# hkbharath/MARL-MASS

Hardware: AMD Instinct MI355X
Metric: agent-steps/sec (whole node), MASS CBF shield on, 65536 envs x 8 CAVs (higher is better)
Workload: dtype f64

## Files before the change

### include/mm_qp.h

```cpp
#ifndef MM_QP_H
#define MM_QP_H

#ifndef MMM_FN
#define MMM_FN static inline
#endif

#define MM_QP_MAXITERS 100
#define MM_QP_ABSTOL 1e-7
#define MM_QP_RELTOL 1e-6
#define MM_QP_FEASTOL 1e-7
#define MM_QP_STEP 0.99
#define MM_QP_FEASTOL_SQ 0x1.6849b86a12b9bp-47

#ifndef MM_QP_RCP
#define MM_QP_RCP(b) (b)
#define MM_QP_DIVR(a, b, R) ((a) / (b))
#endif
#ifndef MM_QP_DIV
#define MM_QP_DIV(a, b) ((a) / (b))
#endif
#ifndef MM_QP_SQRT
#define MM_QP_SQRT(x) sqrt(x)
#endif

typedef struct MMQpKkt {
  double g0, g3;
  double l00, l20, l22;
  double r00, r22;
  double di0, di1, di2, di3;
} MMQpKkt;

typedef struct MMQpState {
  double a, h0, h1, h2, h3, resz0;
  double x0, x2, gap;
  double s0, s1, s2, s3, z0, z1, z2, z3;
  double d0, d1, d2, d3, di0, di1, di2, di3;
  double l0, l1, l2, l3;
  double ax0, ax2;
  int m4, iters;
} MMQpState;
typedef struct MMQpRes { double rx0, rx2, rz0, rz1, rz2, rz3; } MMQpRes;

MMM_FN int mm_qp_factor(MMQpKkt *f, double a, int m4, double di0, double di1, double di2, double di3) {
  f->di0 = di0; f->di1 = di1; f->di2 = di2; f->di3 = 0.0;
  f->g0 = di0 * a;
  f->g3 = 0.0;
  double s00 = f->g0 * f->g0 + di1 * di1 + di2 * di2;
  double s20 = 0.0 + (-di0) * f->g0;
  double s22 = di0 * di0;
  if (m4) {
    f->di3 = di3;
    f->g3 = di3 * a;
    s00 = s00 + f->g3 * f->g3;
    s20 = s20 + (-di3) * f->g3;
    s22 = s22 + di3 * di3;
  }
  s00 = s00 + 1.0;
  s22 = s22 + 1e18;
  if (!(s00 > 0.0)) return 0;
  f->l00 = MM_QP_SQRT(s00);
  f->r00 = MM_QP_RCP(f->l00);
  f->l20 = MM_QP_DIVR(s20, f->l00, f->r00);
  const double t = s22 - f->l20 * f->l20;
  if (!(t > 0.0)) return 0;
  f->l22 = MM_QP_SQRT(t);
  f->r22 = MM_QP_RCP(f->l22);
  return 1;
}
MMM_FN void mm_qp_solve(const MMQpKkt *f, int m4, double *x0, double *x2, double *z0, double *z1, double *z2, double *z3) {
  double w0 = *z0 * f->di0, w1 = *z1 * f->di1, w2 = *z2 * f->di2, w3 = 0.0;
  double t = 0.0 + f->g0 * w0;
  t = t + f->di1 * w1;
  t = t + (-f->di2) * w2;
  double u = 0.0 + (-f->di0) * w0;
  if (m4) {
    w3 = *z3 * f->di3;
    t = t + f->g3 * w3;
    u = u + (-f->di3) * w3;
  }
  double a0 = *x0 + t;
  double a2 = *x2 + u;
  a0 = MM_QP_DIVR(a0, f->l00, f->r00);
  a2 = a2 - a0 * f->l20;
  a2 = MM_QP_DIVR(a2, f->l22, f->r22);
  a2 = MM_QP_DIVR(a2, f->l22, f->r22);
  t = a0 - f->l20 * a2;
  a0 = MM_QP_DIVR(t, f->l00, f->r00);
  t = -w0; t = t + a0 * f->g0; t = t + a2 * (-f->di0); *z0 = t;
  t = -w1; t = t + a0 * f->di1; *z1 = t;
  t = -w2; t = t + a0 * (-f->di2); *z2 = t;
  if (m4) { t = -w3; t = t + a0 * f->g3; t = t + a2 * (-f->di3); *z3 = t; }
  *x0 = a0; *x2 = a2;
}
MMM_FN double mm_qp_dot(double p0, double q0, double p1, double q1, double p2, double q2, double p3, double q3, int m4) {
  double t = 0.0 + p0 * q0;
  t = t + p1 * q1;
  t = t + p2 * q2;
  if (m4) t = t + p3 * q3;
  return t;
}
MMM_FN double mm_qp_maxneg(double p0, double p1, double p2, double p3, int m4) {
  double t = -p0;
  if (-p1 > t) t = -p1;
  if (-p2 > t) t = -p2;
  if (m4 && -p3 > t) t = -p3;
  return t;
}

MMM_FN int mm_qp_start(MMQpState *q, double a, double h0, double h1, double h2, double h3, int rows) {
  const int m4 = rows == 4;
  q->a = a; q->m4 = m4; q->iters = 0;
  q->ax0 = q->ax2 = INFINITY;
  q->h0 = h0; q->h1 = h1; q->h2 = h2; q->h3 = m4 ? h3 : 0.0;
  q->resz0 = fmax(1.0, sqrt(mm_qp_dot(q->h0, q->h0, q->h1, q->h1, q->h2, q->h2, q->h3, q->h3, m4)));
  q->d0 = q->d1 = q->d2 = q->d3 = 1.0; q->di0 = q->di1 = q->di2 = q->di3 = 1.0; q->l0 = q->l1 = q->l2 = q->l3 = 1.0;
  MMQpKkt kkt;
  if (!mm_qp_factor(&kkt, a, m4, 1.0, 1.0, 1.0, 1.0)) {
    q->x0 = a - a + (h0 - h0); q->x2 = q->x0; q->gap = q->x0;
    q->s0 = q->s1 = q->s2 = q->s3 = q->z0 = q->z1 = q->z2 = q->z3 = q->x0;
    return 0;
  }
  double x0 = -0.0, x2 = -0.0;
  double z0 = q->h0, z1 = q->h1, z2 = q->h2, z3 = q->h3;
  mm_qp_solve(&kkt, m4, &x0, &x2, &z0, &z1, &z2, &z3);
  double s0 = -z0, s1 = -z1, s2 = -z2, s3 = -z3;
  const double ts = mm_qp_maxneg(s0, s1, s2, s3, m4);
  int shift = ts >= 0.0;
  if (!shift) shift = ts >= -1e-8 * fmax(sqrt(mm_qp_dot(s0, s0, s1, s1, s2, s2, s3, s3, m4)), 1.0);
  if (shift) { const double sh = 1.0 + ts; s0 = s0 + sh; s1 = s1 + sh; s2 = s2 + sh; s3 = s3 + sh; }
  const double tz = mm_qp_maxneg(z0, z1, z2, z3, m4);
  shift = tz >= 0.0;
  if (!shift) shift = tz >= -1e-8 * fmax(sqrt(mm_qp_dot(z0, z0, z1, z1, z2, z2, z3, z3, m4)), 1.0);
  if (shift) { const double sh = 1.0 + tz; z0 = z0 + sh; z1 = z1 + sh; z2 = z2 + sh; z3 = z3 + sh; }
  q->x0 = x0; q->x2 = x2;
  q->s0 = s0; q->s1 = s1; q->s2 = s2; q->s3 = s3; q->z0 = z0; q->z1 = z1; q->z2 = z2; q->z3 = z3;
  q->gap = mm_qp_dot(s0, z0, s1, z1, s2, z2, s3, z3, m4);
  return 1;
}

#ifndef MM_QP_ILOGB
#define MM_QP_ILOGB(x) ilogb(x)
#define MM_QP_LDEXP(x, e) ldexp(x, e)
#define MM_QP_RINT(x) rint(x)
#endif
MMM_FN int mm_qp_row_state(double s, double z, double rz, double hmag) {
  if (rz == 0.0 && s <= 0x1p-70 * hmag && s >= 0x1p-400 && z >= 0x1p+20) return 1;
  if (z <= 0x1p-60) return 2;
  return 0;
}
MMM_FN int mm_qp_frozen(const MMQpState *q, const MMQpRes *r) {
  if (q->iters < 16 || !(q->a > 0.0)) return 0;
  if (!(fabs(q->ax0) <= 0x1p-75 * fabs(q->x0)) || !(fabs(q->ax2) <= 0x1p-75 * fabs(q->x2))) return 0;
// ... 49 lines not shown
    }
  }
#ifdef MM_QP_CERTIFY
  if (!met && mm_qp_frozen(q, r)) return 3;
#endif
  return met ? 1 : 0;
}

#define MM_QP_PASS(I)                                                                                              \
  {                                                                                                                \
    double t0_ = 0.0, t1_ = 0.0, t2_ = 0.0, t3_ = 0.0;                                                             \
    if (I == 1) { t0_ = t0_ - ws0; t1_ = t1_ - ws1; t2_ = t2_ - ws2; }                                             \
    t0_ = t0_ - lsq0; t1_ = t1_ - lsq1; t2_ = t2_ - lsq2;                                                          \
    ds0 = t0_ + sigma * mu; ds1 = t1_ + sigma * mu; ds2 = t2_ + sigma * mu;                                        \
    dx0 = -r->rx0; dx2 = -r->rx2;                                                                                  \
    ds0 = MM_QP_DIVR(ds0, q->l0, rl0); ds1 = MM_QP_DIVR(ds1, q->l1, rl1); ds2 = MM_QP_DIVR(ds2, q->l2, rl2);       \
    dz0 = -r->rz0 - q->d0 * ds0; dz1 = -r->rz1 - q->d1 * ds1; dz2 = -r->rz2 - q->d2 * ds2;                         \
    if (m4) {                                                                                                      \
      if (I == 1) t3_ = t3_ - ws3;                                                                                 \
      t3_ = t3_ - lsq3;                                                                                            \
      ds3 = t3_ + sigma * mu;                                                                                      \
      ds3 = MM_QP_DIVR(ds3, q->l3, rl3);                                                                           \
      dz3 = -r->rz3 - q->d3 * ds3;                                                                                 \
    }                                                                                                              \
    mm_qp_solve(&kkt, m4, &dx0, &dx2, &dz0, &dz1, &dz2, &dz3);                                                     \
    ds0 = ds0 - dz0; ds1 = ds1 - dz1; ds2 = ds2 - dz2;                                                             \
    if (m4) ds3 = ds3 - dz3;                                                                                       \
    dsdz = mm_qp_dot(ds0, dz0, ds1, dz1, ds2, dz2, ds3, dz3, m4);                                                  \
    if (I == 0) { ws0 = ds0 * dz0; ws1 = ds1 * dz1; ws2 = ds2 * dz2; if (m4) ws3 = ds3 * dz3; }                    \
    ds0 = MM_QP_DIVR(ds0, q->l0, rl0); dz0 = MM_QP_DIVR(dz0, q->l0, rl0);                                          \
    ds1 = MM_QP_DIVR(ds1, q->l1, rl1); dz1 = MM_QP_DIVR(dz1, q->l1, rl1);                                          \
    ds2 = MM_QP_DIVR(ds2, q->l2, rl2); dz2 = MM_QP_DIVR(dz2, q->l2, rl2);                                          \
    if (m4) { ds3 = MM_QP_DIVR(ds3, q->l3, rl3); dz3 = MM_QP_DIVR(dz3, q->l3, rl3); }                              \
    const double ts_ = mm_qp_maxneg(ds0, ds1, ds2, ds3, m4), tz_ = mm_qp_maxneg(dz0, dz1, dz2, dz3, m4);           \
    const double tm_ = fmax(0.0, fmax(ts_, tz_));                                                                  \
    if (tm_ == 0) step = 1.0;                                                                                      \
    else if (I == 0) step = fmin(1.0, MM_QP_DIV(1.0, tm_));                                                        \
    else step = fmin(1.0, MM_QP_DIV(MM_QP_STEP, tm_));                                                             \
  }
#define MM_QP_UPDATE(K)                                                                                            \
  {                                                                                                                \
    double us_ = (step * ds##K + 1.0) * q->l##K, uz_ = (step * dz##K + 1.0) * q->l##K;                            \
    us_ = MM_QP_SQRT(us_);                                                                                         \
    uz_ = MM_QP_SQRT(uz_);                                                                                         \
    q->d##K = MM_QP_DIV(q->d##K * us_, uz_);                                                                       \
    q->di##K = MM_QP_DIV(1.0, q->d##K);                                                                            \
    q->l##K = us_ * uz_;                                                                                           \
    q->s##K = q->d##K * q->l##K;                                                                                   \
    q->z##K = q->di##K * q->l##K;                                                                                  \
  }
#define MM_QP_SCALE0(K)                                                                                            \
  { q->d##K = MM_QP_SQRT(MM_QP_DIV(q->s##K, q->z##K)); q->di##K = MM_QP_DIV(1.0, q->d##K); q->l##K = MM_QP_SQRT(q->s##K * q->z##K); }

MMM_FN int mm_qp_bottom(MMQpState *q, const MMQpRes *r) {
  const int m4 = q->m4;
  const double a = q->a, mm = m4 ? 4.0 : 3.0, gap = q->gap;
  if (q->iters == 0) {
    MM_QP_SCALE0(0) MM_QP_SCALE0(1) MM_QP_SCALE0(2)
    if (m4) MM_QP_SCALE0(3)
  }
  const double lsq0 = q->l0 * q->l0, lsq1 = q->l1 * q->l1, lsq2 = q->l2 * q->l2;
  const double rl0 = MM_QP_RCP(q->l0), rl1 = MM_QP_RCP(q->l1), rl2 = MM_QP_RCP(q->l2);
  double lsq3 = 1.0, rl3 = 1.0;
  if (m4) { lsq3 = q->l3 * q->l3; rl3 = MM_QP_RCP(q->l3); }
  (void)rl0; (void)rl1; (void)rl2; (void)rl3;
  MMQpKkt kkt;
  if (!mm_qp_factor(&kkt, a, m4, q->di0, q->di1, q->di2, q->di3)) return 0;
  const double mu = gap / mm;
  double sigma = 0.0, step = 1.0, dx0 = 0.0, dx2 = 0.0, dsdz = 0.0;
  double ds0 = 0.0, ds1 = 0.0, ds2 = 0.0, ds3 = 0.0, dz0 = 0.0, dz1 = 0.0, dz2 = 0.0, dz3 = 0.0;
  double ws0 = 0.0, ws1 = 0.0, ws2 = 0.0, ws3 = 0.0;
  MM_QP_PASS(0)
  {
    const double sg = fmin(1.0, fmax(0.0, 1.0 - step + MM_QP_DIV(dsdz, gap) * (step * step)));
    sigma = sg * sg * sg;
  }
  MM_QP_PASS(1)
  q->ax0 = step * dx0;
  q->ax2 = step * dx2;
  q->x0 = q->x0 + q->ax0;
  q->x2 = q->x2 + q->ax2;
  MM_QP_UPDATE(0) MM_QP_UPDATE(1) MM_QP_UPDATE(2)
  if (m4) MM_QP_UPDATE(3)
  q->gap = mm_qp_dot(q->l0, q->l0, q->l1, q->l1, q->l2, q->l2, q->l3, q->l3, m4);
  q->iters = q->iters + 1;
  return 1;
}

MMM_FN int mm_qp_ipm_cbf(double a, double h0, double h1, double h2, double h3, int rows, double *d_out, double *s_out,
                         int *iters_out) {
  MMQpState q;
  MMQpRes r;
  int status = 0, certified = 0;
  (void)certified;
  if (mm_qp_start(&q, a, h0, h1, h2, h3, rows)) {
    for (;;) {
      const int stop = mm_qp_top(&q, &r);
      if (stop) { status = stop == 1; certified = stop == 3; break; }
      if (!mm_qp_bottom(&q, &r)) break;
    }
  }
  *d_out = q.x0; *s_out = q.x2; *iters_out = q.iters;
#ifdef MM_QP_CERTIFY
  if (certified) *iters_out = MM_QP_MAXITERS;
#endif
  return status;
}

#endif
```

### marl-mass_amd/csrc/mm_device.h

```cpp
#pragma once
#include <hip/hip_runtime.h>
#include <stdint.h>

#include "../../include/mm_abi.h"

#define MM_DEV __device__ __forceinline__
#define MMM_FN __device__ __forceinline__
#include "../../include/mm_math.h"
#ifndef MM_QP_NO_CERTIFY
#define MM_QP_CERTIFY
#endif
#include "../../include/mm_qp.h"

namespace mm {

#ifndef MM_TRIG_SELECTS
#define MM_TRIG_SELECTS 1
#endif
#ifndef MM_ATAN_SELECTS
#define MM_ATAN_SELECTS 1
#endif
#ifndef MM_CORNER_SELECTS
#define MM_CORNER_SELECTS 1
#endif
#ifndef MM_CLIP_SELECTS
#define MM_CLIP_SELECTS 1
#endif
constexpr bool kTrigSelects = MM_TRIG_SELECTS != 0, kAtanSelects = MM_ATAN_SELECTS != 0;
constexpr bool kCornerSelects = MM_CORNER_SELECTS != 0, kClipSelects = MM_CLIP_SELECTS != 0;
// ... 225 lines not shown
```

### marl-mass_amd/csrc/mm_div.h

```cpp
#pragma once
#include "mm_device.h"

namespace mm {

MM_DEV double rcp_rn(double d) {
  double y = __builtin_amdgcn_rcp(d);
  double e = fma(-d, y, 1.0);
  y = fma(e, y, y);
  e = fma(-d, y, 1.0);
  y = fma(e, y, y);
  e = fma(-d, y, 1.0);
  return fma(e, y, y);
}
MM_DEV bool rcp_ok(double d) {
  const double ad = fabs(d);
  const unsigned lo = (unsigned)__double2loint(d);
  return (ad >= 0x1p-400) & (ad <= 0x1p400) & (lo != 0xffffffffu);
}
MM_DEV bool num_ok(double x) {
  const double ax = fabs(x);
  return (ax <= 0x1p400) & ((ax >= 0x1p-400) | (x == 0.0));
}
MM_DEV double div_g(double x, double d, double y, bool d_ok, bool need = true) {
  const double q = x * y;
// ... 8 lines not shown
}
MM_DEV double rcp_g(double d, double y, bool d_ok) {
  if (__builtin_expect(__any(!d_ok), 0)) {
    const double s = 1.0 / d;
    y = d_ok ? y : s;
  }
  return y;
}
MM_DEV double div_n(double x, int n, bool need = true) {
  constexpr double kRcp[17] = {0.0,      1.0 / 1,  1.0 / 2,  1.0 / 3,  1.0 / 4,  1.0 / 5,  1.0 / 6,  1.0 / 7, 1.0 / 8,
                               1.0 / 9,  1.0 / 10, 1.0 / 11, 1.0 / 12, 1.0 / 13, 1.0 / 14, 1.0 / 15, 1.0 / 16};
  const bool n_ok = (unsigned)(n - 1) < 16u;
  return div_g(x, (double)n, kRcp[n_ok ? n : 0], n_ok, need);
}

}
```

### marl-mass_amd/csrc/mm_kernels.hip

```cpp
#pragma once
#include <hip/hip_runtime.h>
#include <math.h>
#include <stdio.h>
#include <string.h>

#include <type_traits>

#include "mm_device.h"
#include "mm_div.h"
#include "mm_handle.h"
#include "mm_relation.h"
#define MM_COUNTS_FN __host__ __device__ inline
#include "../../include/mm_counts.h"
#include "../../include/mm_policy_wide.h"
#include "../../include/mm_env_params.h"

using namespace mm;

struct DevCfg {
  int env_kind, shield, nsub, T, action_masking, auto_reset, obs_f64, N, E, debug_flags, n_hdv;
  double dt, collision_reward, high_speed_reward, headway_cost, headway_time, merging_lane_cost;
  double rs_lo, rs_hi, eta, tau;
  double inv_dt, rs_span, rs_ispan, rs_span2, rs_ispan2;
  int agent_reward;
// ... 839 lines not shown
  if (!MASS) {
    veto = !lc_allowed;
  } else {
    veto = s.can_abort_lc && !lc_allowed;
    if (!veto && (v.hl == 2 || v.hl == 0) && v.v < kStoppingSpeed) us0 = s.u0;
    if (inv_lona >= -1e-6) fl |= MM_FLAG_COLLABORATE_ADJ;
    else fl &= ~MM_FLAG_COLLABORATE_ADJ;
  }
  if (!veto) fl |= MM_FLAG_IS_LC_SAFE;
  o.acc = div_c(us0 - s.evx, dt, c.inv_dt);
  o.us0 = us0; o.veto = veto; o.flags = fl;
  o.qt.rows = s.cadj ? 4 : 3; o.qt.a = s.g0; o.qt.h0 = r.h0; o.qt.h1 = s.h1; o.qt.h2 = s.h2; o.qt.h3 = r.h3; o.qt.d = d;
  o.qt.margin = fmin(fmin(s.hls_lona, inv_lona), fmin(s.hls_lonr, inv_lonr));
  return o;
}
template <bool MASS, bool PRE = false, bool IPM = false>
MM_DEV ShieldOut shield_dyn(const DevCfg &c, const Veh &v, const ShieldStatic &s, const Neigh &nb, bool run_qp = true) {
  const ShieldRows r = shield_rows<PRE>(c, s, nb);
  double d;
  bool optimal = true;
  if constexpr (IPM) {
    d = 0.0;
    if (run_qp) {
      double slack;
      int iters;
      optimal = mm_qp_ipm_cbf(s.g0, r.h0, s.h1, s.h2, r.h3, s.cadj ? 4 : 3, &d, &slack, &iters) != 0;
    }
  } else {
    d = qp_exact(s, r);
  }
  return shield_post<MASS>(c, v, s, r, d, optimal, IPM && run_qp);
}
template <bool MASS, bool PRE = false, bool IPM = false>
MM_DEV ShieldOut shield_eval(const DevCfg &c, const Veh &v, double cpsi, int pk_self, const Neigh &nb, bool run_qp = true) {
  const ShieldStatic s = shield_static<MASS>(c, v, cpsi, pk_self, nb);
  return shield_dyn<MASS, PRE, IPM>(c, v, s, nb, run_qp);
}

struct Rel {
  double key;
  int cls;
  bool cflag;
};
MM_DEV Rel relate_word(double ex, double ey, int epk, bool other, double ox, double oy, int opk, int esh) {
  const bool o_hdv = false;
  const int elane = epk & 7, enl = (epk >> 3) & 7, olane = opk & 7;
  Rel r;
  const double dx = ox - ex, dy = oy - ey;
  const bool close = other & ((dx * dx + dy * dy) < kT180);
  const double esx = lane_sx(elane);
  const double ld = (ox - esx) - (ex - esx);
// ... 138 lines not shown
    q.d0 = q.d1 = q.d2 = q.d3 = q.di0 = q.di1 = q.di2 = q.di3 = q.l0 = q.l1 = q.l2 = q.l3 = 1.0;
    q.ax0 = q.ax2 = 0; q.m4 = 0; q.iters = 0;
  }
#ifdef MM_STAMPS
  unsigned long long _t_last = __builtin_amdgcn_s_memtime(), _t_acc = 0;
#endif
  int since = 0;
  bool serve = false;
  bool urgent = phase != PH_DONE && sb.urgent[e] != 0, slow_now = false;
  constexpr int VQ_CAP = NV <= 8 ? 16 : 1;
  __shared__ double s_vq[VQ_CAP][40];
  __shared__ int s_vq_own[VQ_CAP], s_redo[64];
  s_redo[ln] = 0;
  int vq_head = 0, vq_tail = 0;
  constexpr bool kSpec = MASS && NV <= 8 && !MIXED;
  bool nospec = !kSpec || (c.debug_flags & 32) != 0;
  int help_owner = 0;
  double help_pred = 0.0;
  for (int trip = 0;; trip++) {
    SCOUNT(4);
    if (trip > 3 * (MM_QP_MAXITERS + 3 + MM_SWEEP_GATE_W) * (NV + 1)) { atomicOr(c.err, MM_LATCH_INTERNAL); break; }
    bool push = false;
    if (phase == PH_RUN) {
      const int stop = mm_qp_top(&q, &rs);
      {
        if (stop || sing) { phase = PH_FIN; opt = stop == 1 && !sing; }
        else if (kSpec && q.iters == MM_SWEEP_SPEC_AT && !nospec && q.a > 0.0) {
          const double hc = (q.m4 && q.h3 < q.h0) ? q.h3 : q.h0, sstar = (-q.a * q.h2) - hc;
          if (q.h2 > 1e-3 && sstar > 1e-4) {
            const int ex = ilogb(q.a * 1e18 * sstar) - 2;
// ... 166 lines not shown
                }
              }
            }
          }
          const int s_ol = nb.has_ol ? j_ol : 0, s_oa = nb.has_oa ? j_oa : 0, s_oar = nb.has_oar ? j_oar : 0;
          nb.ol_x = s_w[W_HX][s_ol][ln]; nb.ol_gu = s_w[W_GU][s_ol][ln];
          nb.oa_x = s_w[W_HX][s_oa][ln]; nb.oa_gu = s_w[W_GU][s_oa][ln];
          nb.oar_x = s_w[W_X][s_oar][ln]; nb.oar_vx = s_w[W_VX][s_oar][ln];
          nb.ol_vx = nb.oa_vx = nb.ol_acc = nb.ol_g = nb.oa_acc = nb.oa_g = 0;
          obstacle_override<MASS>(nb, ex, ey);
          Veh v;
          v.x = ex; v.v = e_v; v.gvx = e_gvx; v.act_acc = e_acc;
          ss = shield_static<MASS>(c, v, cpsi, epk, nb);
          rw = shield_rows<true>(c, ss, nb);
          sing = false;
          int stop = mm_qp_start(&q, ss.g0, rw.h0, ss.h1, ss.h2, rw.h3, ss.cadj ? 4 : 3) != 0 ? 0 : 2;
          if (!stop) stop = mm_qp_top(&q, &rs);
          phase = stop == 0 ? PH_RUN : PH_FIN;
          opt = stop == 1;
        }
      }
    }
    SSTAMP(2);
    if (!__any(phase != PH_DONE)) {
      const int nq = kSpec ? vq_tail - vq_head : 0;
      if (kSpec && nq > 0) {
        __builtin_amdgcn_fence(__ATOMIC_ACQUIRE, "wavefront");
        bool helping = ln < nq;
        if (helping) {
          const double *t = s_vq[(vq_head + ln) % VQ_CAP];
          q.a = t[0]; q.h0 = t[1]; q.h1 = t[2]; q.h2 = t[3]; q.h3 = t[4]; q.resz0 = t[5]; q.x0 = t[6]; q.x2 = t[7]; q.gap = t[8];
          q.s0 = t[9]; q.s1 = t[10]; q.s2 = t[11]; q.s3 = t[12]; q.z0 = t[13]; q.z1 = t[14]; q.z2 = t[15]; q.z3 = t[16];
          q.d0 = t[17]; q.d1 = t[18]; q.d2 = t[19]; q.d3 = t[20]; q.di0 = t[21]; q.di1 = t[22]; q.di2 = t[23]; q.di3 = t[24];
          q.l0 = t[25]; q.l1 = t[26]; q.l2 = t[27]; q.l3 = t[28]; q.ax0 = t[29]; q.ax2 = t[30];
          rs.rx0 = t[31]; rs.rx2 = t[32]; rs.rz0 = t[33]; rs.rz1 = t[34]; rs.rz2 = t[35]; rs.rz3 = t[36];
          help_pred = t[37];
          const int mi = (int)t[38];
          q.m4 = mi & 1; q.iters = mi >> 1;
          help_owner = s_vq_own[(vq_head + ln) % VQ_CAP];
        }
        vq_head = vq_tail;
        while (__any(helping)) {
          if (helping) {
            const bool ok = mm_qp_bottom(&q, &rs) != 0;
            const int stop = ok ? mm_qp_top(&q, &rs) : 2;
            if (stop) {
              if (stop == 1 || __double_as_longlong(q.x0) != __double_as_longlong(help_pred)) s_redo[help_owner] = 1;
              helping = false;
            }
          }
        }
        __builtin_amdgcn_fence(__ATOMIC_RELEASE, "wavefront");
        __builtin_amdgcn_wave_barrier();
      }
      __builtin_amdgcn_fence(__ATOMIC_ACQUIRE, "wavefront");
      const bool redo = kSpec && s_redo[ln] != 0;
      if (!kSpec || !__any(redo)) break;
      if (redo) {
#ifdef MM_STAMPS
        atomicAdd(&g_stamps_s[blockIdx.x % 4096 * 8 + 6], 1ull);
#endif
        s_redo[ln] = 0;
        reload_views();
        r = 0; dirty = (c.debug_flags & 1) != 0; nospec = true;
        phase = PH_SETUP;
      }
      continue;
    }
    if (__any(phase == PH_RUN)) {
      if (phase == PH_RUN) sing = mm_qp_bottom(&q, &rs) == 0;
    }
    SSTAMP(3);
  }
  if (e < c.E) sb.urgent[e] = slow_now ? 1 : 0;
#ifdef MM_STAMPS
  if ((threadIdx.x & 63) < 8 && blockIdx.x < 4096) g_stamps_s[blockIdx.x * 8 + (threadIdx.x & 63)] += _t_acc;
#endif
}

#ifndef MM_MIN_WAVES
#define MM_MIN_WAVES 2
#endif
#ifndef MM_NONE_WAVES
#define MM_NONE_WAVES 3
#endif
// ... 42 lines not shown
  constexpr bool MASS = (SHIELD == MM_SHIELD_MASS);
  static_assert(!IPM || SHIELDED, "the IPM mode lives in shielded kernels");
  static_assert(!SPLIT || IPM, "the split form exists for the interior-point kernels");
  static_assert(!PENV || (SHIELDED && KIND == MM_ENV_V1 && !TRACE && !SPLIT), "per-env parameters: fused shielded v1 kernels without the trace");
#ifdef MM_SERIAL_ALL
  constexpr bool kSerialOnly = true || IPM;
#else
#ifdef MM_SERIAL_MASS
  constexpr bool kSerialOnly = MIXED || MASS || IPM;
#else
  constexpr bool kSerialOnly = MIXED;
#endif
#endif
  constexpr bool kSine = SHIELDED && !SPLIT && !MIXED && !IPM && !kSerialOnly && kPow2<G> && G <= 8;
  constexpr bool kScan = kScanSelects && !MIXED && !TRACE;
#ifndef MM_CARRY_POSE
#define MM_CARRY_POSE 1
#endif
  constexpr bool kCarry = kSine && MM_CARRY_POSE != 0;
#ifndef MM_PRIMARY_PRIOR
#define MM_PRIMARY_PRIOR 1
#endif
  constexpr bool kPrimary = kSine && !TRACE && kVetoPrior && MM_PRIMARY_PRIOR != 0;
#ifndef MM_SINE_CARRY
#define MM_SINE_CARRY 0
#endif
  constexpr bool kSineCarry = kPrimary && MM_SINE_CARRY != 0;
#ifndef MM_ACT_FRAME
#define MM_ACT_FRAME 1
#endif
// ... 574 lines not shown
                da = shfl_d(gu_cur, src_ol); db = shfl_d(gu_cur, src_oa);
                const unsigned long long fm = __ballot(fin);
                ready = ready && (!ol_dyn || ((fm >> src_ol) & 1ull)) && (!oa_dyn || ((fm >> src_oa) & 1ull));
              }
              if (__any(ready)) {
                if (ready) {
                  if (MASS) { if (ol_dyn) nb.ol_gu = da; if (oa_dyn) nb.oa_gu = db; }
                  const ShieldRows rw = shield_rows<true>(c, ss, nb);
                  const int rows = ss.cadj ? 4 : 3;
                  if ((qc_meta & 7) == rows && __double_as_longlong(qc_h0) == __double_as_longlong(rw.h0) &&
                      __double_as_longlong(qc_h3) == __double_as_longlong(rw.h3)) {
                    q.x0 = qc_d; late = true; late_opt = (qc_meta & 8) != 0;
                  } else {
                    qc_h0 = rw.h0; qc_h3 = rw.h3;
                    sing = false;
                    int stop = mm_qp_start(&q, ss.g0, rw.h0, ss.h1, ss.h2, rw.h3, rows) != 0 ? 0 : 2;
                    if (!stop) stop = mm_qp_top(&q, &rs);
                    run = stop == 0;
                    if (stop) { late = true; late_opt = stop == 1; }
                  }
                }
              }
              const bool any_run = __any(run);
              if (any_run) {
                if (run) sing = mm_qp_bottom(&q, &rs) == 0;
              }
              more = any_run || __any(!fin);
            }
            if (shield_on) so = shield_post<MASS>(env_cfg<PENV>(c, e, st.E), v, ss, shield_rows<true>(c, ss, nb), qc_d, (qc_meta & 8) != 0, true);
          } else {
          if constexpr (MASS && kRoundsLite) {
            const bool slow_lc = (v.hl == 2 || v.hl == 0) && v.v < kStoppingSpeed;
            ShieldRows rr;
            double d_cur = 0.0;
            if constexpr (kRoundsPrior) {
              if (shield_on) acc_cur = rounds_seed(c, ss);
            }
#ifdef MM_STAMPS
            {
              STAMP(4);
// ... 161 lines not shown
          if (has_tw) f_oa = f_tw & ~1u;
          Neigh nb;
          nb.has_ol = f_ol != none; nb.has_oa = f_oa != none; nb.has_oar = f_oar != none;
          const int s_ol = gb + (nb.has_ol ? (int)((f_ol >> 1) & 15u) : 0);
          const int s_oa = gb + (nb.has_oa ? (int)((f_oa >> 1) & 15u) : 0);
          const int s_oar = gb + (nb.has_oar ? (int)((f_oar >> 1) & 15u) : 0);
          nb.ol_x = shfl_d(whx, s_ol); nb.ol_gu = shfl_d(wgu, s_ol);
          nb.oa_x = shfl_d(whx, s_oa); nb.oa_gu = shfl_d(wgu, s_oa);
          nb.ol_vx = nb.oa_vx = nb.ol_acc = nb.ol_g = nb.oa_acc = nb.oa_g = 0;
          nb.oar_x = shfl_d(wx, s_oar); nb.oar_vx = shfl_d(wvx, s_oar);
          nb.constrain_adj = MASS && nb.has_oa && (f_oa & 1u);
          bool hss_collab = false;
          if (has_tw) { nb.constrain_adj = MASS; hss_collab = !MASS; }
          obstacle_override<MASS>(nb, v.x, v.y);
          const bool mine = has && a == ai && shield_on;
          ShieldOut s1 = shield_eval<MASS, true, IPM>(env_cfg<PENV>(c, e, st.E), v, cpsi, kHBits ? pk_self & 0xFF : pk_self, nb, mine);
          if (hss_collab) s1.flags |= MM_FLAG_IS_COLLABORATING;
          if (IPM && mine && s1.bounds) atomicOr(c.err, MM_LATCH_QP_BOUNDS);
          if (mine) {
            new_acc = s1.acc; veto = s1.veto; new_flags = s1.flags; qt = s1.qt;
            if (TRACE) trace_status(out.trace + (long long)k * MM_T_COUNT * A + i, A, s1);
            use_B = veto && needB;
            const Cand cc = chosen(use_B);
            double nv = v.v + new_acc * dt;
            nv = nv > 0 ? nv : 0;
            wx = cc.x; wy = cc.y; wh = cc.h; wg = cc.gvx; wacc = new_acc; wvx = nv * cc.cpsi;
            whx = s_cold[C_H1X][tid]; whvx = s_cold[C_H1VX][tid]; wpk = cc.pk;
            wgu = slot_gu<MASS>(whvx, MASS ? wacc : kCbfAccLo, wg, dt);
          }
        }
        if (MIXED && hdv && twin_shift != 0 && w_stepped) s_cold[C_H1X][tid] = whx;
// ... 555 lines not shown
```

### marl-mass_amd/csrc/mm_main.hip

```cpp
#include "mm_step_host.h"

__global__ void qp_kernel(int n, const double *__restrict__ G, const double *__restrict__ h,
                          const int32_t *__restrict__ rows, int solver, double *__restrict__ u, uint8_t *status,
                          int32_t *iters, int *err) {
  const int k = blockIdx.x * blockDim.x + threadIdx.x;
  if (k >= n) return;
  const double *g = G + (long long)k * 12, *hh = h + (long long)k * 4;
  const int m = rows[k];
  bool ok = (m == 3 || m == 4) && g[1] == 0.0 && g[2] == -1.0 && g[3] == 1.0 && g[4] == 0.0 && g[5] == 0.0 && g[6] == -1.0 &&
            g[7] == 0.0 && g[8] == 0.0;
  if (ok && m == 4) ok = g[9] == g[0] && g[10] == 0.0 && g[11] == -1.0;
  if (iters) iters[k] = 0;
  if (!ok) {
    u[k * 3 + 0] = u[k * 3 + 1] = u[k * 3 + 2] = __builtin_nan("");
    if (status) status[k] = MM_QPS_BAD_STRUCTURE;
    atomicOr(err, MM_LATCH_BAD_QP);
    return;
  }
  const double a = g[0];
  if (solver == MM_QP_IPM) {
    double d, sl;
    int it;
    const int opt = mm_qp_ipm_cbf(a, hh[0], hh[1], hh[2], m == 4 ? hh[3] : 0.0, m, &d, &sl, &it);
    u[k * 3 + 0] = d; u[k * 3 + 1] = 0.0; u[k * 3 + 2] = sl;
// ... 739 lines not shown
```

Measured before the change: 2.753 billion.

## Use guarded reciprocal-multiply divisions in early QP iterations with exact fallback

Adds a fast path to the IPM QP solver. For the first iterations, divisions are replaced by a shared reciprocal plus one FMA correction step, and operand exponents are tracked in a guard flag. If any lane's guard trips, or once the iteration count passes a threshold, the wave redoes the Newton step or start with the exact literal divisions. This cuts the cost of f64 divides in the CBF shield solver, at the price of more code, register pressure and possible redundant recomputation when guards trip. The path is enabled for MASS spec-queue kernels, while the main step kernel keeps it off; it also adds launch bounds to qp_kernel.

After: 2.750 billion. About the same (-0.1%).

```diff
diff --git a/include/mm_qp.h b/include/mm_qp.h
--- a/include/mm_qp.h
+++ b/include/mm_qp.h
@@ -21,6 +21,23 @@
 #endif
 #ifndef MM_QP_SQRT
 #define MM_QP_SQRT(x) sqrt(x)
+#endif
+#ifndef MM_QP_FAST_ITERS
+#define MM_QP_FAST_ITERS 13
+#endif
+#ifdef MM_QP_FAST
+#define MM_QP_FARGS , const int fast, MM_QP_FLAG_T *flag
+#define MM_QP_FPASS , fast, flag
+#define MM_QP_RCP_(b) (fast ? MM_QP_FAST_RCP(b, *flag) : MM_QP_RCP(b))
+#define MM_QP_DIVR_(a, b, R) (fast ? MM_QP_FAST_DIVR(a, b, R, *flag) : MM_QP_DIVR(a, b, R))
+#ifndef MM_QP_REDO_NOTE
+#define MM_QP_REDO_NOTE(block)
+#endif
+#else
+#define MM_QP_FARGS
+#define MM_QP_FPASS
+#define MM_QP_RCP_(b) MM_QP_RCP(b)
+#define MM_QP_DIVR_(a, b, R) MM_QP_DIVR(a, b, R)
 #endif
 
 typedef struct MMQpKkt {
@@ -41,7 +58,7 @@
 } MMQpState;
 typedef struct MMQpRes { double rx0, rx2, rz0, rz1, rz2, rz3; } MMQpRes;
 
-MMM_FN int mm_qp_factor(MMQpKkt *f, double a, int m4, double di0, double di1, double di2, double di3) {
+MMM_FN int mm_qp_factor(MMQpKkt *f, double a, int m4, double di0, double di1, double di2, double di3 MM_QP_FARGS) {
   f->di0 = di0; f->di1 = di1; f->di2 = di2; f->di3 = 0.0;
   f->g0 = di0 * a;
   f->g3 = 0.0;
@@ -59,15 +76,15 @@
   s22 = s22 + 1e18;
   if (!(s00 > 0.0)) return 0;
   f->l00 = MM_QP_SQRT(s00);
-  f->r00 = MM_QP_RCP(f->l00);
-  f->l20 = MM_QP_DIVR(s20, f->l00, f->r00);
+  f->r00 = MM_QP_RCP_(f->l00);
+  f->l20 = MM_QP_DIVR_(s20, f->l00, f->r00);
   const double t = s22 - f->l20 * f->l20;
   if (!(t > 0.0)) return 0;
   f->l22 = MM_QP_SQRT(t);
-  f->r22 = MM_QP_RCP(f->l22);
+  f->r22 = MM_QP_RCP_(f->l22);
   return 1;
 }
-MMM_FN void mm_qp_solve(const MMQpKkt *f, int m4, double *x0, double *x2, double *z0, double *z1, double *z2, double *z3) {
+MMM_FN void mm_qp_solve(const MMQpKkt *f, int m4, double *x0, double *x2, double *z0, double *z1, double *z2, double *z3 MM_QP_FARGS) {
   double w0 = *z0 * f->di0, w1 = *z1 * f->di1, w2 = *z2 * f->di2, w3 = 0.0;
   double t = 0.0 + f->g0 * w0;
   t = t + f->di1 * w1;
@@ -80,12 +97,12 @@
   }
   double a0 = *x0 + t;
   double a2 = *x2 + u;
-  a0 = MM_QP_DIVR(a0, f->l00, f->r00);
+  a0 = MM_QP_DIVR_(a0, f->l00, f->r00);
   a2 = a2 - a0 * f->l20;
-  a2 = MM_QP_DIVR(a2, f->l22, f->r22);
-  a2 = MM_QP_DIVR(a2, f->l22, f->r22);
+  a2 = MM_QP_DIVR_(a2, f->l22, f->r22);
+  a2 = MM_QP_DIVR_(a2, f->l22, f->r22);
   t = a0 - f->l20 * a2;
-  a0 = MM_QP_DIVR(t, f->l00, f->r00);
+  a0 = MM_QP_DIVR_(t, f->l00, f->r00);
   t = -w0; t = t + a0 * f->g0; t = t + a2 * (-f->di0); *z0 = t;
   t = -w1; t = t + a0 * f->di1; *z1 = t;
   t = -w2; t = t + a0 * (-f->di2); *z2 = t;
@@ -107,7 +124,7 @@
   return t;
 }
 
-MMM_FN int mm_qp_start(MMQpState *q, double a, double h0, double h1, double h2, double h3, int rows) {
+MMM_FN int mm_qp_start_form(MMQpState *q, double a, double h0, double h1, double h2, double h3, int rows MM_QP_FARGS) {
   const int m4 = rows == 4;
   q->a = a; q->m4 = m4; q->iters = 0;
   q->ax0 = q->ax2 = INFINITY;
@@ -115,14 +132,14 @@
   q->resz0 = fmax(1.0, sqrt(mm_qp_dot(q->h0, q->h0, q->h1, q->h1, q->h2, q->h2, q->h3, q->h3, m4)));
   q->d0 = q->d1 = q->d2 = q->d3 = 1.0; q->di0 = q->di1 = q->di2 = q->di3 = 1.0; q->l0 = q->l1 = q->l2 = q->l3 = 1.0;
   MMQpKkt kkt;
-  if (!mm_qp_factor(&kkt, a, m4, 1.0, 1.0, 1.0, 1.0)) {
+  if (!mm_qp_factor(&kkt, a, m4, 1.0, 1.0, 1.0, 1.0 MM_QP_FPASS)) {
     q->x0 = a - a + (h0 - h0); q->x2 = q->x0; q->gap = q->x0;
     q->s0 = q->s1 = q->s2 = q->s3 = q->z0 = q->z1 = q->z2 = q->z3 = q->x0;
     return 0;
   }
   double x0 = -0.0, x2 = -0.0;
   double z0 = q->h0, z1 = q->h1, z2 = q->h2, z3 = q->h3;
-  mm_qp_solve(&kkt, m4, &x0, &x2, &z0, &z1, &z2, &z3);
+  mm_qp_solve(&kkt, m4, &x0, &x2, &z0, &z1, &z2, &z3 MM_QP_FPASS);
   double s0 = -z0, s1 = -z1, s2 = -z2, s3 = -z3;
   const double ts = mm_qp_maxneg(s0, s1, s2, s3, m4);
   int shift = ts >= 0.0;
@@ -136,6 +153,29 @@
   q->s0 = s0; q->s1 = s1; q->s2 = s2; q->s3 = s3; q->z0 = z0; q->z1 = z1; q->z2 = z2; q->z3 = z3;
   q->gap = mm_qp_dot(s0, z0, s1, z1, s2, z2, s3, z3, m4);
   return 1;
+}
+MMM_FN int mm_qp_start_literal(MMQpState *q, double a, double h0, double h1, double h2, double h3, int rows) {
+#ifdef MM_QP_FAST
+  MM_QP_FLAG_T flag = MM_QP_FLAG_INIT;
+  return mm_qp_start_form(q, a, h0, h1, h2, h3, rows, 0, &flag);
+#else
+  return mm_qp_start_form(q, a, h0, h1, h2, h3, rows);
+#endif
+}
+MMM_FN int mm_qp_start(MMQpState *q, double a, double h0, double h1, double h2, double h3, int rows) {
+#ifdef MM_QP_FAST
+  MM_QP_FLAG_T flag = MM_QP_FLAG_INIT;
+  int ok = mm_qp_start_form(q, a, h0, h1, h2, h3, rows, 1, &flag);
+  if (MM_QP_ANY(MM_QP_FLAG_SET(flag))) {
+    if (MM_QP_FLAG_SET(flag)) {
+      MM_QP_REDO_NOTE(0);
+      ok = mm_qp_start_form(q, a, h0, h1, h2, h3, rows, 0, &flag);
+    }
+  }
+  return ok;
+#else
+  return mm_qp_start_form(q, a, h0, h1, h2, h3, rows);
+#endif
 }
 
 #ifndef MM_QP_ILOGB
@@ -215,24 +255,24 @@
     t0_ = t0_ - lsq0; t1_ = t1_ - lsq1; t2_ = t2_ - lsq2;                                                          \
     ds0 = t0_ + sigma * mu; ds1 = t1_ + sigma * mu; ds2 = t2_ + sigma * mu;                                        \
     dx0 = -r->rx0; dx2 = -r->rx2;                                                                                  \
-    ds0 = MM_QP_DIVR(ds0, q->l0, rl0); ds1 = MM_QP_DIVR(ds1, q->l1, rl1); ds2 = MM_QP_DIVR(ds2, q->l2, rl2);       \
+    ds0 = MM_QP_DIVR_(ds0, q->l0, rl0); ds1 = MM_QP_DIVR_(ds1, q->l1, rl1); ds2 = MM_QP_DIVR_(ds2, q->l2, rl2);       \
     dz0 = -r->rz0 - q->d0 * ds0; dz1 = -r->rz1 - q->d1 * ds1; dz2 = -r->rz2 - q->d2 * ds2;                         \
     if (m4) {                                                                                                      \
       if (I == 1) t3_ = t3_ - ws3;                                                                                 \
       t3_ = t3_ - lsq3;                                                                                            \
       ds3 = t3_ + sigma * mu;                                                                                      \
-      ds3 = MM_QP_DIVR(ds3, q->l3, rl3);                                                                           \
+      ds3 = MM_QP_DIVR_(ds3, q->l3, rl3);                                                                           \
       dz3 = -r->rz3 - q->d3 * ds3;                                                                                 \
     }                                                                                                              \
-    mm_qp_solve(&kkt, m4, &dx0, &dx2, &dz0, &dz1, &dz2, &dz3);                                                     \
+    mm_qp_solve(&kkt, m4, &dx0, &dx2, &dz0, &dz1, &dz2, &dz3 MM_QP_FPASS);                                                  \
     ds0 = ds0 - dz0; ds1 = ds1 - dz1; ds2 = ds2 - dz2;                                                             \
     if (m4) ds3 = ds3 - dz3;                                                                                       \
     dsdz = mm_qp_dot(ds0, dz0, ds1, dz1, ds2, dz2, ds3, dz3, m4);                                                  \
     if (I == 0) { ws0 = ds0 * dz0; ws1 = ds1 * dz1; ws2 = ds2 * dz2; if (m4) ws3 = ds3 * dz3; }                    \
-    ds0 = MM_QP_DIVR(ds0, q->l0, rl0); dz0 = MM_QP_DIVR(dz0, q->l0, rl0);                                          \
-    ds1 = MM_QP_DIVR(ds1, q->l1, rl1); dz1 = MM_QP_DIVR(dz1, q->l1, rl1);                                          \
-    ds2 = MM_QP_DIVR(ds2, q->l2, rl2); dz2 = MM_QP_DIVR(dz2, q->l2, rl2);                                          \
-    if (m4) { ds3 = MM_QP_DIVR(ds3, q->l3, rl3); dz3 = MM_QP_DIVR(dz3, q->l3, rl3); }                              \
+    ds0 = MM_QP_DIVR_(ds0, q->l0, rl0); dz0 = MM_QP_DIVR_(dz0, q->l0, rl0);                                          \
+    ds1 = MM_QP_DIVR_(ds1, q->l1, rl1); dz1 = MM_QP_DIVR_(dz1, q->l1, rl1);                                          \
+    ds2 = MM_QP_DIVR_(ds2, q->l2, rl2); dz2 = MM_QP_DIVR_(dz2, q->l2, rl2);                                          \
+    if (m4) { ds3 = MM_QP_DIVR_(ds3, q->l3, rl3); dz3 = MM_QP_DIVR_(dz3, q->l3, rl3); }                              \
     const double ts_ = mm_qp_maxneg(ds0, ds1, ds2, ds3, m4), tz_ = mm_qp_maxneg(dz0, dz1, dz2, dz3, m4);           \
     const double tm_ = fmax(0.0, fmax(ts_, tz_));                                                                  \
     if (tm_ == 0) step = 1.0;                                                                                      \
@@ -253,7 +293,53 @@
 #define MM_QP_SCALE0(K)                                                                                            \
   { q->d##K = MM_QP_SQRT(MM_QP_DIV(q->s##K, q->z##K)); q->di##K = MM_QP_DIV(1.0, q->d##K); q->l##K = MM_QP_SQRT(q->s##K * q->z##K); }
 
-MMM_FN int mm_qp_bottom(MMQpState *q, const MMQpRes *r) {
+typedef struct MMQpStep { double dx0, dx2, ds0, ds1, ds2, ds3, dz0, dz1, dz2, dz3, step; } MMQpStep;
+MMM_FN void mm_qp_scale0(MMQpState *q) {
+  MM_QP_SCALE0(0) MM_QP_SCALE0(1) MM_QP_SCALE0(2)
+  if (q->m4) MM_QP_SCALE0(3)
+}
+MMM_FN int mm_qp_newton(const MMQpState *q, const MMQpRes *r, MMQpStep *o MM_QP_FARGS) {
+  const int m4 = q->m4;
+  const double a = q->a, mm = m4 ? 4.0 : 3.0, gap = q->gap;
+  const double lsq0 = q->l0 * q->l0, lsq1 = q->l1 * q->l1, lsq2 = q->l2 * q->l2;
+  const double rl0 = MM_QP_RCP_(q->l0), rl1 = MM_QP_RCP_(q->l1), rl2 = MM_QP_RCP_(q->l2);
+  double lsq3 = 1.0, rl3 = 1.0;
+  if (m4) { lsq3 = q->l3 * q->l3; rl3 = MM_QP_RCP_(q->l3); }
+  (void)rl0; (void)rl1; (void)rl2; (void)rl3;
+  MMQpKkt kkt;
+  if (!mm_qp_factor(&kkt, a, m4, q->di0, q->di1, q->di2, q->di3 MM_QP_FPASS)) return 0;
+  const double mu = gap / mm;
+  double sigma = 0.0, step = 1.0, dx0 = 0.0, dx2 = 0.0, dsdz = 0.0;
+  double ds0 = 0.0, ds1 = 0.0, ds2 = 0.0, ds3 = 0.0, dz0 = 0.0, dz1 = 0.0, dz2 = 0.0, dz3 = 0.0;
+  double ws0 = 0.0, ws1 = 0.0, ws2 = 0.0, ws3 = 0.0;
+  MM_QP_PASS(0)
+  {
+    const double sg = fmin(1.0, fmax(0.0, 1.0 - step + MM_QP_DIV(dsdz, gap) * (step * step)));
+    sigma = sg * sg * sg;
+  }
+  MM_QP_PASS(1)
+  o->dx0 = dx0; o->dx2 = dx2; o->step = step;
+  o->ds0 = ds0; o->ds1 = ds1; o->ds2 = ds2; o->ds3 = ds3; o->dz0 = dz0; o->dz1 = dz1; o->dz2 = dz2; o->dz3 = dz3;
+  return 1;
+}
+MMM_FN void mm_qp_update(MMQpState *q, const MMQpStep *o) {
+  const int m4 = q->m4;
+  const double step = o->step, dx0 = o->dx0, dx2 = o->dx2;
+  const double ds0 = o->ds0, ds1 = o->ds1, ds2 = o->ds2, ds3 = o->ds3, dz0 = o->dz0, dz1 = o->dz1, dz2 = o->dz2, dz3 = o->dz3;
+  q->ax0 = step * dx0;
+  q->ax2 = step * dx2;
+  q->x0 = q->x0 + q->ax0;
+  q->x2 = q->x2 + q->ax2;
+  MM_QP_UPDATE(0) MM_QP_UPDATE(1) MM_QP_UPDATE(2)
+  if (m4) MM_QP_UPDATE(3)
+  q->gap = mm_qp_dot(q->l0, q->l0, q->l1, q->l1, q->l2, q->l2, q->l3, q->l3, m4);
+  q->iters = q->iters + 1;
+}
+MMM_FN int mm_qp_bottom_literal(MMQpState *q, const MMQpRes *r) {
+#ifdef MM_QP_FAST
+  const int fast = 0;
+  MM_QP_FLAG_T flag_ = MM_QP_FLAG_INIT, *flag = &flag_;
+#endif
   const int m4 = q->m4;
   const double a = q->a, mm = m4 ? 4.0 : 3.0, gap = q->gap;
   if (q->iters == 0) {
@@ -261,12 +347,12 @@
     if (m4) MM_QP_SCALE0(3)
   }
   const double lsq0 = q->l0 * q->l0, lsq1 = q->l1 * q->l1, lsq2 = q->l2 * q->l2;
-  const double rl0 = MM_QP_RCP(q->l0), rl1 = MM_QP_RCP(q->l1), rl2 = MM_QP_RCP(q->l2);
+  const double rl0 = MM_QP_RCP_(q->l0), rl1 = MM_QP_RCP_(q->l1), rl2 = MM_QP_RCP_(q->l2);
   double lsq3 = 1.0, rl3 = 1.0;
-  if (m4) { lsq3 = q->l3 * q->l3; rl3 = MM_QP_RCP(q->l3); }
+  if (m4) { lsq3 = q->l3 * q->l3; rl3 = MM_QP_RCP_(q->l3); }
   (void)rl0; (void)rl1; (void)rl2; (void)rl3;
   MMQpKkt kkt;
-  if (!mm_qp_factor(&kkt, a, m4, q->di0, q->di1, q->di2, q->di3)) return 0;
+  if (!mm_qp_factor(&kkt, a, m4, q->di0, q->di1, q->di2, q->di3 MM_QP_FPASS)) return 0;
   const double mu = gap / mm;
   double sigma = 0.0, step = 1.0, dx0 = 0.0, dx2 = 0.0, dsdz = 0.0;
   double ds0 = 0.0, ds1 = 0.0, ds2 = 0.0, ds3 = 0.0, dz0 = 0.0, dz1 = 0.0, dz2 = 0.0, dz3 = 0.0;
@@ -287,18 +373,47 @@
   q->iters = q->iters + 1;
   return 1;
 }
-
-MMM_FN int mm_qp_ipm_cbf(double a, double h0, double h1, double h2, double h3, int rows, double *d_out, double *s_out,
-                         int *iters_out) {
+MMM_FN int mm_qp_bottom(MMQpState *q, const MMQpRes *r) {
+#ifdef MM_QP_FAST
+  MMQpStep o;
+  MM_QP_FLAG_T flag = MM_QP_FLAG_INIT;
+  if (q->iters == 0) mm_qp_scale0(q);
+  const int late = MM_QP_ANY(q->iters >= MM_QP_FAST_ITERS);
+  int ok = 0;
+  if (!late) ok = mm_qp_newton(q, r, &o, 1, &flag);
+  if (late || MM_QP_ANY(MM_QP_FLAG_SET(flag))) {
+    if (late || MM_QP_FLAG_SET(flag)) {
+      if (!late) { MM_QP_REDO_NOTE(1); }
+      ok = mm_qp_newton(q, r, &o, 0, &flag);
+    }
+  }
+  if (!ok) return 0;
+  mm_qp_update(q, &o);
+  return 1;
+#else
+  return mm_qp_bottom_literal(q, r);
+#endif
+}
+
+MMM_FN int mm_qp_ipm_cbf_form(double a, double h0, double h1, double h2, double h3, int rows, double *d_out, double *s_out,
+                              int *iters_out, const int literal) {
   MMQpState q;
   MMQpRes r;
   int status = 0, certified = 0;
   (void)certified;
-  if (mm_qp_start(&q, a, h0, h1, h2, h3, rows)) {
+#ifdef MM_QP_FAST
+#define MM_QP_START_(q, a, h0, h1, h2, h3, rows) (literal ? mm_qp_start_literal(q, a, h0, h1, h2, h3, rows) : mm_qp_start(q, a, h0, h1, h2, h3, rows))
+#define MM_QP_BOTTOM_(q, r) (literal ? mm_qp_bottom_literal(q, r) : mm_qp_bottom(q, r))
+#else
+#define MM_QP_START_(q, a, h0, h1, h2, h3, rows) mm_qp_start(q, a, h0, h1, h2, h3, rows)
+#define MM_QP_BOTTOM_(q, r) mm_qp_bottom(q, r)
+  (void)literal;
+#endif
+  if (MM_QP_START_(&q, a, h0, h1, h2, h3, rows)) {
     for (;;) {
       const int stop = mm_qp_top(&q, &r);
       if (stop) { status = stop == 1; certified = stop == 3; break; }
-      if (!mm_qp_bottom(&q, &r)) break;
+      if (!MM_QP_BOTTOM_(&q, &r)) break;
     }
   }
   *d_out = q.x0; *s_out = q.x2; *iters_out = q.iters;
@@ -307,5 +422,9 @@
 #endif
   return status;
 }
-
-#endif
+MMM_FN int mm_qp_ipm_cbf(double a, double h0, double h1, double h2, double h3, int rows, double *d_out, double *s_out,
+                         int *iters_out) {
+  return mm_qp_ipm_cbf_form(a, h0, h1, h2, h3, rows, d_out, s_out, iters_out, 0);
+}
+
+#endif
diff --git a/marl-mass_amd/csrc/mm_device.h b/marl-mass_amd/csrc/mm_device.h
--- a/marl-mass_amd/csrc/mm_device.h
+++ b/marl-mass_amd/csrc/mm_device.h
@@ -10,9 +10,31 @@
 #ifndef MM_QP_NO_CERTIFY
 #define MM_QP_CERTIFY
 #endif
+#ifndef MM_QP_SHARED_RCP
+#define MM_QP_SHARED_RCP 1
+#endif
+#include "mm_div.h"
+#if MM_QP_SHARED_RCP
+#define MM_QP_FAST
+#define MM_QP_FLAG_T unsigned
+#define MM_QP_FLAG_INIT 0u
+#define MM_QP_FLAG_SET(flag) ::mm::guard_raised(flag)
+#define MM_QP_ANY(cond) __builtin_expect(__any(cond), 0)
+#define MM_QP_FAST_RCP(b, flag) ::mm::rcp_s((b), (flag))
+#define MM_QP_FAST_DIVR(a, b, R, flag) ::mm::div_s((a), (b), (R), (flag))
+#endif
 #include "../../include/mm_qp.h"
 
 namespace mm {
+
+template <bool FAST> MM_DEV int qp_start(MMQpState *q, double a, double h0, double h1, double h2, double h3, int rows) {
+  if constexpr (FAST) return mm_qp_start(q, a, h0, h1, h2, h3, rows);
+  else return mm_qp_start_literal(q, a, h0, h1, h2, h3, rows);
+}
+template <bool FAST> MM_DEV int qp_bottom(MMQpState *q, const MMQpRes *r) {
+  if constexpr (FAST) return mm_qp_bottom(q, r);
+  else return mm_qp_bottom_literal(q, r);
+}
 
 #ifndef MM_TRIG_SELECTS
 #define MM_TRIG_SELECTS 1
diff --git a/marl-mass_amd/csrc/mm_div.h b/marl-mass_amd/csrc/mm_div.h
--- a/marl-mass_amd/csrc/mm_div.h
+++ b/marl-mass_amd/csrc/mm_div.h
@@ -1,5 +1,9 @@
 #pragma once
-#include "mm_device.h"
+#include <hip/hip_runtime.h>
+
+#ifndef MM_DEV
+#define MM_DEV __device__ __forceinline__
+#endif
 
 namespace mm {
 
@@ -46,4 +50,23 @@
   return div_g(x, (double)n, kRcp[n_ok ? n : 0], n_ok, need);
 }
 
+
+constexpr unsigned kGuardExpLo = 1023 - 400, kGuardExpSpan = 800;
+MM_DEV unsigned guard_term(double v) { return (((unsigned)__double2hiint(v) >> 20) & 0x7ffu) - kGuardExpLo; }
+MM_DEV bool guard_raised(unsigned flag) { return flag > kGuardExpSpan; }
+MM_DEV void num_s(double x, unsigned &flag) { flag = max(flag, guard_term(x)); }
+MM_DEV void den_s(double d, unsigned &flag) {
+  const unsigned t = (unsigned)__double2loint(d) == 0xffffffffu ? 0xffffffffu : guard_term(d);
+  flag = max(flag, t);
 }
+MM_DEV double rcp_s(double d, unsigned &flag) {
+  den_s(d, flag);
+  return rcp_rn(d);
+}
+MM_DEV double div_s(double x, double d, double y, unsigned &flag) {
+  num_s(x, flag);
+  const double q = x * y;
+  return fma(fma(-q, d, x), y, q);
+}
+
+}
diff --git a/marl-mass_amd/csrc/mm_kernels.hip b/marl-mass_amd/csrc/mm_kernels.hip
--- a/marl-mass_amd/csrc/mm_kernels.hip
+++ b/marl-mass_amd/csrc/mm_kernels.hip
@@ -877,7 +877,7 @@
   o.qt.margin = fmin(fmin(s.hls_lona, inv_lona), fmin(s.hls_lonr, inv_lonr));
   return o;
 }
-template <bool MASS, bool PRE = false, bool IPM = false>
+template <bool MASS, bool PRE = false, bool IPM = false, bool QPFAST = true>
 MM_DEV ShieldOut shield_dyn(const DevCfg &c, const Veh &v, const ShieldStatic &s, const Neigh &nb, bool run_qp = true) {
   const ShieldRows r = shield_rows<PRE>(c, s, nb);
   double d;
@@ -887,17 +887,17 @@
     if (run_qp) {
       double slack;
       int iters;
-      optimal = mm_qp_ipm_cbf(s.g0, r.h0, s.h1, s.h2, r.h3, s.cadj ? 4 : 3, &d, &slack, &iters) != 0;
+      optimal = mm_qp_ipm_cbf_form(s.g0, r.h0, s.h1, s.h2, r.h3, s.cadj ? 4 : 3, &d, &slack, &iters, !QPFAST) != 0;
     }
   } else {
     d = qp_exact(s, r);
   }
   return shield_post<MASS>(c, v, s, r, d, optimal, IPM && run_qp);
 }
-template <bool MASS, bool PRE = false, bool IPM = false>
+template <bool MASS, bool PRE = false, bool IPM = false, bool QPFAST = true>
 MM_DEV ShieldOut shield_eval(const DevCfg &c, const Veh &v, double cpsi, int pk_self, const Neigh &nb, bool run_qp = true) {
   const ShieldStatic s = shield_static<MASS>(c, v, cpsi, pk_self, nb);
-  return shield_dyn<MASS, PRE, IPM>(c, v, s, nb, run_qp);
+  return shield_dyn<MASS, PRE, IPM, QPFAST>(c, v, s, nb, run_qp);
 }
 
 struct Rel {
@@ -1066,6 +1066,7 @@
   s_redo[ln] = 0;
   int vq_head = 0, vq_tail = 0;
   constexpr bool kSpec = MASS && NV <= 8 && !MIXED;
+  constexpr bool kQpFast = MASS || (NV <= 8 && !MIXED);
   bool nospec = !kSpec || (c.debug_flags & 32) != 0;
   int help_owner = 0;
   double help_pred = 0.0;
@@ -1262,7 +1263,7 @@
           ss = shield_static<MASS>(c, v, cpsi, epk, nb);
           rw = shield_rows<true>(c, ss, nb);
           sing = false;
-          int stop = mm_qp_start(&q, ss.g0, rw.h0, ss.h1, ss.h2, rw.h3, ss.cadj ? 4 : 3) != 0 ? 0 : 2;
+          int stop = qp_start<kQpFast>(&q, ss.g0, rw.h0, ss.h1, ss.h2, rw.h3, ss.cadj ? 4 : 3) != 0 ? 0 : 2;
           if (!stop) stop = mm_qp_top(&q, &rs);
           phase = stop == 0 ? PH_RUN : PH_FIN;
           opt = stop == 1;
@@ -1290,7 +1291,7 @@
         vq_head = vq_tail;
         while (__any(helping)) {
           if (helping) {
-            const bool ok = mm_qp_bottom(&q, &rs) != 0;
+            const bool ok = qp_bottom<kQpFast>(&q, &rs) != 0;
             const int stop = ok ? mm_qp_top(&q, &rs) : 2;
             if (stop) {
               if (stop == 1 || __double_as_longlong(q.x0) != __double_as_longlong(help_pred)) s_redo[help_owner] = 1;
@@ -1316,7 +1317,7 @@
       continue;
     }
     if (__any(phase == PH_RUN)) {
-      if (phase == PH_RUN) sing = mm_qp_bottom(&q, &rs) == 0;
+      if (phase == PH_RUN) sing = qp_bottom<kQpFast>(&q, &rs) == 0;
     }
     SSTAMP(3);
   }
@@ -1389,6 +1390,7 @@
 #endif
   constexpr bool kSine = SHIELDED && !SPLIT && !MIXED && !IPM && !kSerialOnly && kPow2<G> && G <= 8;
   constexpr bool kScan = kScanSelects && !MIXED && !TRACE;
+  constexpr bool kQpFast = false;
 #ifndef MM_CARRY_POSE
 #define MM_CARRY_POSE 1
 #endif
@@ -1993,7 +1995,7 @@
                   } else {
                     qc_h0 = rw.h0; qc_h3 = rw.h3;
                     sing = false;
-                    int stop = mm_qp_start(&q, ss.g0, rw.h0, ss.h1, ss.h2, rw.h3, rows) != 0 ? 0 : 2;
+                    int stop = qp_start<kQpFast>(&q, ss.g0, rw.h0, ss.h1, ss.h2, rw.h3, rows) != 0 ? 0 : 2;
                     if (!stop) stop = mm_qp_top(&q, &rs);
                     run = stop == 0;
                     if (stop) { late = true; late_opt = stop == 1; }
@@ -2002,7 +2004,7 @@
               }
               const bool any_run = __any(run);
               if (any_run) {
-                if (run) sing = mm_qp_bottom(&q, &rs) == 0;
+                if (run) sing = qp_bottom<kQpFast>(&q, &rs) == 0;
               }
               more = any_run || __any(!fin);
             }
@@ -2194,7 +2196,7 @@
           if (has_tw) { nb.constrain_adj = MASS; hss_collab = !MASS; }
           obstacle_override<MASS>(nb, v.x, v.y);
           const bool mine = has && a == ai && shield_on;
-          ShieldOut s1 = shield_eval<MASS, true, IPM>(env_cfg<PENV>(c, e, st.E), v, cpsi, kHBits ? pk_self & 0xFF : pk_self, nb, mine);
+          ShieldOut s1 = shield_eval<MASS, true, IPM, kQpFast>(env_cfg<PENV>(c, e, st.E), v, cpsi, kHBits ? pk_self & 0xFF : pk_self, nb, mine);
           if (hss_collab) s1.flags |= MM_FLAG_IS_COLLABORATING;
           if (IPM && mine && s1.bounds) atomicOr(c.err, MM_LATCH_QP_BOUNDS);
           if (mine) {
diff --git a/marl-mass_amd/csrc/mm_main.hip b/marl-mass_amd/csrc/mm_main.hip
--- a/marl-mass_amd/csrc/mm_main.hip
+++ b/marl-mass_amd/csrc/mm_main.hip
@@ -1,6 +1,6 @@
 #include "mm_step_host.h"
 
-__global__ void qp_kernel(int n, const double *__restrict__ G, const double *__restrict__ h,
+__global__ __launch_bounds__(256) void qp_kernel(int n, const double *__restrict__ G, const double *__restrict__ h,
                           const int32_t *__restrict__ rows, int solver, double *__restrict__ u, uint8_t *status,
                           int32_t *iters, int *err) {
   const int k = blockIdx.x * blockDim.x + threadIdx.x;
```
